# QEC-project-2020/MCMC-QEC-toric-RL

Measured on AMD Instinct MI355X. Metric: MCMC sweeps/sec (whole node), L=9 toric p=0.15; eq-class histogram match, higher is better.
Workload: dtype u8

## Files before the change

mcmc-qec-toric-rl_amd/csrc/ladder_wu.hpp:

```cpp
#pragma once
#include "ladder_kernel.hpp"
#include "shortest_book.hpp"
#include "wu_frames.hpp"

namespace qecmc {

constexpr uint32_t kWuPickStream = 0x800u;
constexpr uint32_t kSubWuPick = 9u, kSubWuAcc = 10u, kSubWuRefine = 11u;

#ifndef QECMC_WU_PRIO_SHIFT
#define QECMC_WU_PRIO_SHIFT 4
#endif
constexpr int kWuPrioShift = QECMC_WU_PRIO_SHIFT;
constexpr bool wu_prio_family(int WV, bool ALPHA) { return kWuPrioShift >= 0 && !ALPHA && WV <= 16; }
__device__ __forceinline__ void wu_step_priority(uint32_t t)
{
    constexpr uint32_t SH = kWuPrioShift < 0 ? 0u : (uint32_t)kWuPrioShift;
    uint32_t k;
    asm volatile("s_and_b32 %0, %1, %2\n\t"
                 "s_cmp_lg_u32 %0, 0\n\t"
                 "s_cbranch_scc1 4f\n\t"
                 "s_bfe_u32 %0, %1, %3\n\t"
                 "s_cmp_lg_u32 %0, 0\n\t"
                 "s_cbranch_scc1 1f\n\t"
                 "s_setprio 3\n\t"
                 "s_branch 4f\n"
                 "1:\n\t"
                 "s_cmp_lg_u32 %0, 1\n\t"
                 "s_cbranch_scc1 2f\n\t"
                 "s_setprio 2\n\t"
                 "s_branch 4f\n"
                 "2:\n\t"
                 "s_cmp_lg_u32 %0, 2\n\t"
                 "s_cbranch_scc1 3f\n\t"
                 "s_setprio 1\n\t"
                 "s_branch 4f\n"
                 "3:\n\t"
                 "s_setprio 0\n"
                 "4:"
                 : "=&s"(k) : "s"(t), "n"((1u << SH) - 1u), "n"(SH | (2u << 16)) : "scc");
}

template <int WV> struct WuVec;
template <> struct WuVec<4> { typedef uint32_t type __attribute__((ext_vector_type(4))); };
template <> struct WuVec<8> { typedef uint32_t type __attribute__((ext_vector_type(8))); };
template <> struct WuVec<12> { typedef uint32_t type __attribute__((ext_vector_type(12))); };
template <> struct WuVec<16> { typedef uint32_t type __attribute__((ext_vector_type(16))); };
template <> struct WuVec<32> { typedef uint32_t type __attribute__((ext_vector_type(32))); };

template <int WV> constexpr int wu_base() { return WV == 32 ? 48 : 64 - WV; }
#define WU_BY_WV(M)                                                                                                            \
    if constexpr (WV == 4) { M("{v[60:63]}") } else if constexpr (WV == 8) { M("{v[56:63]}") }                                 \
    else if constexpr (WV == 12) { M("{v[52:63]}") } else if constexpr (WV == 16) { M("{v[48:63]}") }                          \
    else { static_assert(WV == 32, "state widths: 4, 8, 12, 16, 32 words"); M("{v[48:79]}") }
#define WU_EACH(M) M(0) M(1) M(2) M(3) M(4) M(5) M(6) M(7) M(8) M(9) M(10) M(11) M(12) M(13) M(14) M(15) \
                   M(16) M(17) M(18) M(19) M(20) M(21) M(22) M(23) M(24) M(25) M(26) M(27) M(28) M(29) M(30) M(31)

template <int WV> __device__ __forceinline__ void wu_def(typename WuVec<WV>::type &st)
{
#define M(PIN) asm volatile("" : "=" PIN(st));
    WU_BY_WV(M)
#undef M
}
template <int WV> __device__ __forceinline__ void wu_pin(typename WuVec<WV>::type &st)
{
#define M(PIN) asm volatile("" : "+" PIN(st));
    WU_BY_WV(M)
#undef M
}
template <int WV, int w> __device__ __forceinline__ void wu_set(typename WuVec<WV>::type &st, uint32_t v)
{
#define M(PIN) asm volatile("v_mov_b32 v[%c[r]], %[v]" : "+" PIN(st) : [r] "i"(wu_base<WV>() + w), [v] "v"(v));
    WU_BY_WV(M)
#undef M
}
template <int WV, int w> __device__ __forceinline__ uint32_t wu_get(typename WuVec<WV>::type &st)
{
    uint32_t v;
#define M(PIN) asm volatile("v_mov_b32 %[v], v[%c[r]]" : [v] "=v"(v), "+" PIN(st) : [r] "i"(wu_base<WV>() + w));
    WU_BY_WV(M)
#undef M
    return v;
}
template <int WV, int w> __device__ __forceinline__ void wu_xor_s(typename WuVec<WV>::type &st, uint32_t m)
{
// ... 241 lines not shown
    if (xf < ef - band) return true;
    if (xf > ef + band) return false;
    return (double)x * (1.0 / 4294967296.0) < det_exp(y);
}

struct WuAl { uint32_t Dh, any, Nb; };

template <int CODE, int WV>
__device__ __forceinline__ void wu_propose_alpha(const LadderArgs &a, typename WuVec<WV>::type &st, WuAl &al, uint32_t a12, uint32_t cht_addr,
                                                 float lxy, float lz, uint32_t d0, uint32_t d1, uint32_t d2, uint32_t d3,
                                                 uint32_t x0, uint32_t x1, uint32_t x2, uint32_t x3, uint32_t tlo, uint32_t thi, uint32_t omask, uint32_t amask,
                                                 uint64_t refine_k, uint32_t refine_w, uint32_t syn, uint32_t slot, uint32_t m55)
{
    const uint32_t F = wu_read<WV>(st, d0, d1, d2, d3);
    const uint32_t pv = __builtin_amdgcn_perm(thi, tlo, (F & amask) | omask);
    const uint32_t addr = __builtin_amdgcn_sad_u8(pv, 0u, cht_addr);
    const uint32_t dch = *(wu_lds_ptr)(uintptr_t)addr;
    const wu_half2 pD = __builtin_bit_cast(wu_half2, al.Dh) + __builtin_bit_cast(wu_half2, dch);
    const float e = __builtin_amdgcn_exp2f(__builtin_fmaf((float)pD.x, lxy, __builtin_fmaf((float)pD.y, lz, 12.0f)));
    const float dm = e - (float)a12;
    bool acc = dm >= 2.0f;
    if (!acc && dm >= -1.0f) {
        const int nq = a.nq, T1 = nq + 1;
        const double *bt = a.bias_tbl + (size_t)slot * 4 * T1;
        uint32_t nxc = 0;
#define QECMC_WU_CX(w) if constexpr (w < WV) wu_count_x<WV, w>(st, nxc, m55);
        WU_EACH(QECMC_WU_CX)
#undef QECMC_WU_CX
        int dx = 0;
        {
            const uint32_t P0 = x0 >> ((d0 >> 8) & 31u), P1 = x1 >> ((d1 >> 8) & 31u), P2 = x2 >> ((d2 >> 8) & 31u), P3 = x3 >> ((d3 >> 8) & 31u);
            const uint32_t f0 = F & 3u, f1 = (F >> 8) & 3u, f2 = (F >> 16) & 3u, f3 = (F >> 24) & 3u;
            dx += (int)((f0 ^ P0) == 1u) - (int)(f0 == 1u);
            dx += (int)((f1 ^ P1) == 1u) - (int)(f1 == 1u);
            dx += (int)((f2 ^ P2) == 1u) - (int)(f2 == 1u);
            dx += (int)((f3 ^ P3) == 1u) - (int)(f3 == 1u);
        }
        const int bx = (int)(al.Nb & 1023u), bz = (int)((al.Nb >> 10) & 1023u), bxy = (int)(al.Nb >> 20);
        const int cx = (int)nxc + dx, cz = bz + (int)(float)pD.y, cxy = bxy + (int)(float)pD.x;
        const double pn = bt[cx] * bt[T1 + (cxy - cx)] * bt[2 * T1 + cz] * bt[3 * T1 + (nq - cxy - cz)];
        const double pb = bt[bx] * bt[T1 + (bxy - bx)] * bt[2 * T1 + bz] * bt[3 * T1 + (nq - bxy - bz)];
        const double ratio = pn / pb;
        const double ulo = (double)a12 * (1.0 / 4096.0);
        acc = ulo + (1.0 / 4096.0) <= ratio;
        if (!acc && ulo < ratio) {
            const u32x4 rb = wu_philox(refine_k, kSubWuRefine, syn, slot, a.seed_lo, a.seed_hi);
            const uint64_t v44 = ((uint64_t)a12 << 32) | sel4(rb, (int)refine_w);
            acc = (double)v44 * (1.0 / 17592186044416.0) < ratio;
        }
    }
    if (acc) {
        wu_xor<WV>(st, d0, d1, d2, d3, x0, x1, x2, x3);
        al.Dh = __builtin_bit_cast(uint32_t, pD);
        al.any = 1u;
    }
}

template <int CODE>
__device__ __forceinline__ void wu_stage_lds(const LadderArgs &a, uint64_t lad, uint32_t slot, wu_lds_rw xrow, uint32_t &n4, uint32_t &cls, int w0 = 0, int w1 = -1, int rows = 0)
{
    const int NC = a.Nc, W = a.W, L = a.L, nq = a.nq;
    const uint8_t *src = a.resume ? a.states + (lad * NC + slot) * (uint64_t)nq : a.init + (lad / a.replicas) * (uint64_t)nq;
    uint32_t cnt = 0;
    if (w1 < 0) w1 = W;
#pragma unroll 1
    for (int w = w0; w < w1; ++w) {
        uint32_t word = 0;
#pragma unroll 4
        for (int b = 0; b < 16; ++b) {
            const int cell = w * 8 + (b >> 1), q = CODE == kCodeToric ? (cell < L * L ? (b & 1) * L * L + cell : nq) : w * 16 + b;
            if (q < nq) word |= (uint32_t)(src[q] & 3u) << (2 * b);
        }
        xrow[(w - w0) * 64] = word;
        cnt += nnz2(word);
    }
#pragma unroll 1
    for (int r = w1 - w0; r < rows; ++r) xrow[r * 64] = 0u;
    if (w0 != 0) { n4 += 4u * cnt; return; }
    n4 = 4u * cnt;
    cls = (uint32_t)(CODE == kCodeToric ? toric_eq_class_b(L, src) : surf_eq_class_b(CODE, L, src));
    if (CODE == kCodeXzzx) cls = cls == 0 ? 0u : cls == 1 ? 1u : cls == 2 ? 3u : 2u;
}

__device__ __forceinline__ bool wu_pair_flips(const LadderArgs &a, uint32_t car, uint32_t lo, uint32_t x, uint32_t trow, int i)
{
    const int d = (int)(car & 0xFFFFu) - (int)(lo & 0xFFFFu);
    const int dt = d < 0 ? 0 : d > kSwapFast - 1 ? kSwapFast - 1 : d;
    uint32_t thr = *(wu_lds_ptr)(uintptr_t)(trow + 4u * (uint32_t)dt);
    if (__builtin_amdgcn_sicmp(d, kSwapFast - 1, 38) != 0) {
        int il = i, nql = a.nq;
        asm volatile("" : "+s"(il), "+s"(nql));
        const int dg = d < 0 ? 0 : d > nql ? nql : d;
        const uint32_t far = (uint32_t)a.swap_thr[(size_t)il * (size_t)(nql + 1) + (size_t)dg];
        thr = d >= kSwapFast ? far : thr;
    }
    return d <= 0 || x < thr;
}

template <int CODE, int WV, bool CONV, bool QUEUE, bool TOP, int IT, bool ALPHA, bool STATS = false, bool SHORT = false, bool LONG = true>
__device__ __forceinline__ void wu_run(const LadderArgs &a, typename WuVec<WV>::type &st, WuCtx &cx, const WuEnv &ev)
{
    static_assert(!QUEUE || CONV, "the work queue serves the runs that stop by the criterion");
    static_assert(!ALPHA || CODE != kCodeToric, "the alpha rule: xzzx / rotated codes");
    static_assert(!STATS || (!CONV && WV <= 16), "the statistics kernels: fixed-length runs of up to 16 state words");
    static_assert(!SHORT || (CONV && QUEUE && ALPHA && !STATS), "the shortest-chain kernels: the alpha rule's queue kernels");
    [[maybe_unused]] uint32_t swapc = 0, nsum = 0;
    const int L = a.L;
    wu_lds_ptr const lml = (wu_lds_ptr)(uintptr_t)(ev.lds0 + ev.lml_off);
    const uint32_t lds0 = ev.lds0, slot = ev.slot, grp = ev.grp;
    const int lane = ev.lane;
    constexpr bool top = TOP;
    constexpr bool LEAN = !CONV && !ALPHA && WV <= 16;
    constexpr bool FRAME = TOP && wu_frame_steps(WV, CONV, ALPHA, IT) != 0;
    constexpr uint32_t FW = (uint32_t)WV + 1u;
    const uint32_t G = a.n_gen;
    const uint32_t m55 = 0x55555555u;
    uint32_t n4 = cx.n4, cls = cx.cls, flag = cx.flag;
    [[maybe_unused]] uint32_t nef = cx.nef;
    [[maybe_unused]] float lxyf = 0.0f, lzf = 0.0f;
    if constexpr (ALPHA) { lxyf = a.bias_l2f[ev.slot][0]; lzf = a.bias_l2f[ev.slot][1]; }
    [[maybe_unused]] const uint32_t cht_base = ev.lds0 + ev.cht_off;
    uint32_t syn = a.first_syndrome + ev.lad;
    [[maybe_unused]] uint32_t t0 = 0;
    [[maybe_unused]] uint32_t tops0 = cx.tops0, samples = 0;
    const wu_const_ptr desc = (wu_const_ptr)a.wu_desc;
    const uint32_t iters = IT ? (uint32_t)IT : a.iters;
    const uint32_t nch = (iters + 9u) / 10u, nc4 = (iters + 3u) / 4u;
    const uint32_t S = 128u / iters;
    const uint32_t thr16 = (uint32_t)((a.thr_logical + 65535u) >> 16);
    const uint32_t thr_base = lds0 + ev.thr_off;
    uint32_t nbias = 0u - (thr_base + 16u);
    asm volatile("" : "+s"(nbias));
    uint32_t pk = 0;
    [[maybe_unused]] uint32_t pa0 = 0, pa1 = 0, pb0 = 0, pb1 = 0;
    [[maybe_unused]] uint32_t pf_a = 0, pf_b = 0, pf_c = 0, pf_l = 0;
    uint32_t ws = (uint32_t)(a.step0 % S);
    uint64_t wi = a.step0 / S;
    auto refresh = [&]() {
        const u32x4 b = wu_philox(wi * 64u + (uint64_t)lane, kSubWuPick, grp, kWuPickStream + slot, a.seed_lo, a.seed_hi);
        if constexpr (FRAME) {
            constexpr uint32_t FS = (uint32_t)wu_frame_steps(WV, CONV, ALPHA, IT);
            wu_lds_rw const frm = (wu_lds_rw)(uintptr_t)(lds0 + ev.frm_off);
#pragma unroll
            for (uint32_t i = 0; i < (FS * FW + 63u) / 64u; ++i) {
                const uint32_t at = i * 64u + (uint32_t)lane;
                if (at < FS * FW) frm[at] = 0u;
            }
            __builtin_amdgcn_fence(__ATOMIC_ACQ_REL, "wavefront");
            if ((uint32_t)lane < FS * (uint32_t)IT / 2u) {
                wu_lds_rw const row = frm + ((uint32_t)lane / ((uint32_t)IT / 2u)) * FW;
                auto desc_word = [&](uint32_t g, int i) { return a.wu_desc[(size_t)g * (CODE == kCodeToric ? 8u : 16u) + (uint32_t)i]; };
                auto lml_word = [&](uint32_t kind, uint32_t pos, int w) { return lml[(kind * (uint32_t)(L + 1) + pos) * (uint32_t)WV + (uint32_t)w]; };
                auto xor_word = [&](uint32_t w, uint32_t v) { __hip_atomic_fetch_xor(row + w, v, __ATOMIC_RELAXED, __HIP_MEMORY_SCOPE_WORKGROUP); };
                wu_frame_add<CODE, WV>(b.x, b.y, thr16, G, L, desc_word, lml_word, xor_word);
                wu_frame_add<CODE, WV>(b.z, b.w, thr16, G, L, desc_word, lml_word, xor_word);
            }
            __builtin_amdgcn_fence(__ATOMIC_ACQ_REL, "wavefront");
        } else {
        const uint32_t g0 = scale_u32(b.y, G), g1 = scale_u32(b.w, G);
        pk = CODE == kCodeToric ? (g0 << 5) | (g1 << 21) : (g0 << 6) | (g1 << 22);
        if (top) { pa0 = b.x; pb0 = b.y; pa1 = b.z; pb1 = b.w; }
        }
    };
    refresh();
    constexpr bool AHEAD = LEAN && !TOP && IT == 10;
    [[maybe_unused]] u32x4 abn{0, 0, 0, 0};
    if constexpr (AHEAD) abn = wu_philox(a.step0, kSubWuAcc, syn, slot, a.seed_lo, a.seed_hi);

    for (uint64_t t = 0; QUEUE || t < a.nsteps + (CONV ? 1u : 0u); ++t) {
        if constexpr (wu_prio_family(WV, ALPHA)) wu_step_priority((uint32_t)t);
        const uint64_t T = QUEUE ? (uint64_t)((uint32_t)t - t0) : a.step0 + t;
        [[maybe_unused]] uint32_t maskv = 0, cdelta = 0;
        const uint32_t pbase = ws * iters;
        [[maybe_unused]] WuAl al{0u, 0u, 0u};
        if constexpr (ALPHA && !top) al.Nb = wu_counts_packed<WV>(st, m55, a.W);
        if constexpr (FRAME) {
            const uint32_t fv = ((wu_lds_ptr)(uintptr_t)(lds0 + ev.frm_off))[ws * FW + (uint32_t)(lane < WV ? lane : WV)];
            maskv = fv;
            cdelta = (uint32_t)__builtin_amdgcn_readlane((int)fv, WV);
// ... 44 lines not shown
#undef QECMC_WU_LOGICAL
                } else {
                    const uint32_t j = c * 10u + (uint32_t)f;
                    if constexpr (IT == 10) {
                        if constexpr (ALPHA) {
                          if ((f & 1) == 0) {
                            const wu_const_ptr eb = (wu_const_ptr)((wu_const_bytes)desc + (r >> 16));
                            const uint32_t d0 = e[0], d1 = e[1], d2 = e[2], d3 = e[3], x0 = e[4], x1 = e[5], x2 = e[6], x3 = e[7];
                            const uint32_t am = e[11], tlo = e[12], thi = e[13], om = e[14], coff = e[15];
                            const uint32_t b0 = eb[0], b1 = eb[1], b2 = eb[2], b3 = eb[3], y0 = eb[4], y1 = eb[5], y2 = eb[6], y3 = eb[7];
                            const uint32_t an = eb[11], ulo = eb[12], uhi = eb[13], on = eb[14], cofn = eb[15];
                            __builtin_amdgcn_sched_barrier(0);
                            wu_propose_alpha<CODE, WV>(a, st, al, wu_field(ab, f), cht_base + coff, lxyf, lzf, d0, d1, d2, d3, x0, x1, x2, x3, tlo, thi, om, am,
                                                       T * nc4 + (j >> 2), j & 3u, syn, slot, m55);
                            wu_propose_alpha<CODE, WV>(a, st, al, wu_field(ab, f + 1), cht_base + cofn, lxyf, lzf, b0, b1, b2, b3, y0, y1, y2, y3, ulo, uhi, on, an,
                                                       T * nc4 + ((j + 1u) >> 2), (j + 1u) & 3u, syn, slot, m55);
                          }
                        } else if constexpr (CODE == kCodeToric) {
                          if ((f & 1) == 0) {
                            const wu_desc8 da = *(wu_const_desc8)e, db = *(wu_const_desc8)((wu_const_bytes)desc + (r >> 16));
                            __builtin_amdgcn_sched_barrier(0);
                            wu_propose<CODE, WV>(st, n4, wu_field(ab, f), thr_base, nbias, da[0], 0u, da[1], da[2], da[3], 0u, da[4], da[5], da[6], 0u, 0u, 0u,
                                                 T * nc4 + (j >> 2), j & 3u, syn, slot, a.seed_lo, a.seed_hi);
                            wu_propose<CODE, WV>(st, n4, wu_field(ab, f + 1), thr_base, nbias, db[0], 0u, db[1], db[2], db[3], 0u, db[4], db[5], db[6], 0u, 0u, 0u,
                                                 T * nc4 + ((j + 1u) >> 2), (j + 1u) & 3u, syn, slot, a.seed_lo, a.seed_hi);
                          }
                        } else
                        if ((f & 1) == 0) {
                            const wu_const_ptr eb = (wu_const_ptr)((wu_const_bytes)desc + (r >> 16));
                            const uint32_t d0 = e[0], d1 = e[1], d2 = e[2], d3 = e[3], x0 = e[4], x1 = e[5], x2 = e[6], x3 = e[7], tlo = e[8];
                            const uint32_t thi = e[9], om = e[10], am = e[11];
                            const uint32_t b0 = eb[0], b1 = eb[1], b2 = eb[2], b3 = eb[3], y0 = eb[4], y1 = eb[5], y2 = eb[6], y3 = eb[7], ulo = eb[8];
                            const uint32_t uhi = eb[9], on = eb[10], an = eb[11];
                            __builtin_amdgcn_sched_barrier(0);
                            wu_propose<CODE, WV>(st, n4, wu_field(ab, f), thr_base, nbias, d0, d1, d2, d3, x0, x1, x2, x3, tlo, thi, om, am,
                                                 T * nc4 + (j >> 2), j & 3u, syn, slot, a.seed_lo, a.seed_hi);
                            wu_propose<CODE, WV>(st, n4, wu_field(ab, f + 1), thr_base, nbias, b0, b1, b2, b3, y0, y1, y2, y3, ulo, uhi, on, an,
                                                 T * nc4 + ((j + 1u) >> 2), (j + 1u) & 3u, syn, slot, a.seed_lo, a.seed_hi);
                        }
                    } else if constexpr (ALPHA) {
                        const uint32_t d0 = e[0], d1 = e[1], d2 = e[2], d3 = e[3], x0 = e[4], x1 = e[5], x2 = e[6], x3 = e[7];
                        const uint32_t am = e[11], tlo = e[12], thi = e[13], om = e[14], coff = e[15];
                        wu_propose_alpha<CODE, WV>(a, st, al, wu_field(ab, f), cht_base + coff, lxyf, lzf, d0, d1, d2, d3, x0, x1, x2, x3, tlo, thi, om, am,
                                                   T * nc4 + (j >> 2), j & 3u, syn, slot, m55);
                    } else if constexpr (CODE == kCodeToric) {
                        const wu_desc8 d = *(wu_const_desc8)e;
                        wu_propose<CODE, WV>(st, n4, wu_field(ab, f), thr_base, nbias, d[0], 0u, d[1], d[2], d[3], 0u, d[4], d[5], d[6], 0u, 0u, 0u,
                                             T * nc4 + (j >> 2), j & 3u, syn, slot, a.seed_lo, a.seed_hi);
                    } else {
                        const uint32_t d0 = e[0], d1 = e[1], d2 = e[2], d3 = e[3], x0 = e[4], x1 = e[5], x2 = e[6], x3 = e[7], tlo = e[8];
                        const uint32_t thi = e[9], om = e[10], am = e[11];
                        wu_propose<CODE, WV>(st, n4, wu_field(ab, f), thr_base, nbias, d0, d1, d2, d3, x0, x1, x2, x3, tlo, thi, om, am,
                                             T * nc4 + (j >> 2), j & 3u, syn, slot, a.seed_lo, a.seed_hi);
                    }
                }
            }
        }
        if (top) {
            cls ^= cdelta;
            n4 = 0;
            [[maybe_unused]] uint32_t tx = 0, tz = 0, txy = 0;
#define QECMC_WU_FLUSH(w)                                                                                    \
            if constexpr (w < WV) {                                                                          \
                wu_xor_s<WV, w>(st, (uint32_t)__builtin_amdgcn_readlane((int)maskv, w));                     \
                if constexpr (ALPHA) wu_count3<WV, w>(st, tx, tz, txy, m55);                                 \
                else wu_count<WV, w>(st, n4, m55);                                                           \
            }
            WU_EACH(QECMC_WU_FLUSH)
#undef QECMC_WU_FLUSH
            if constexpr (ALPHA) { n4 = tz + txy; nef = tz | (txy << 16); }
            n4 <<= 2;
        } else if constexpr (ALPHA) {
            const wu_half2 D = __builtin_bit_cast(wu_half2, al.Dh);
            const uint32_t ez = (uint32_t)((int)((al.Nb >> 10) & 1023u) + (int)(float)D.y), exy = (uint32_t)((int)(al.Nb >> 20) + (int)(float)D.x);
            n4 = (ez + exy) << 2;
            if (al.any) nef = ez | (exy << 16);
        }
        if (++ws == S) { ws = 0; ++wi; refresh(); }

        if constexpr (LEAN) {
        int NCl = a.Nc, ncl = a.ncls;
        uint32_t slotl = ev.slot, lds0l = ev.lds0, once = a.wu_once;
        asm volatile("" : "+s"(NCl), "+s"(ncl), "+s"(slotl), "+s"(lds0l), "+s"(once));
        if constexpr (STATS) once = 0;
        const int NC = NCl;
        const uint32_t slot = slotl;
        const WuLds ol = wu_lds(NC, WV, ncl, 0, false, false);
        constexpr uint32_t xstride = (uint32_t)WV * 256u;
        const uint32_t xaddr = lds0l + (uint32_t)lane * 4u;
        wu_lds_rw const recl = (wu_lds_rw)(uintptr_t)(xaddr + (uint32_t)ol.rec * 4u), swdl = recl + NC * 64;
        const uint32_t tb0 = lds0l + (uint32_t)ol.swapT * 4u;
        const int swb = NC - 1 - (int)slot;
        constexpr bool TOPDRAWS = !LONG && wu_frame_steps(WV, CONV, ALPHA, IT) != 0;
        u32x4 sb{0, 0, 0, 0};
        [[maybe_unused]] u32x4 sb1{0, 0, 0, 0};
        [[maybe_unused]] bool duty = false;
        if constexpr (TOPDRAWS && TOP) {
            sb = wu_philox(T, 0u, syn, kSwapStream, a.seed_lo, a.seed_hi);
            if (NC > 5) sb1 = wu_philox(T, 1u, syn, kSwapStream, a.seed_lo, a.seed_hi);
        } else if constexpr (!TOPDRAWS) {
            duty = swb >= 0 && swb < 4 && swb * 4 < NC - 1;
            if (duty) sb = wu_philox(T, (uint32_t)swb, syn, kSwapStream, a.seed_lo, a.seed_hi);
        }
        auto put_block = [&](int blk, const u32x4 &v) {
            wu_lds_rw p = swdl + (uint32_t)(blk * 4) * 64u;
            const int left = NC - 1 - blk * 4;
            p[0] = v.x;
            if (left > 1) p[64] = v.y;
            if (left > 2) p[128] = v.z;
            if (left > 3) p[192] = v.w;
        };
        __syncthreads();
        wu_put_all<WV>(st, xaddr + slot * xstride);
        recl[slot * 64u] = pack_info(n4 >> 2, slot, cls, flag);
        if constexpr (TOPDRAWS && TOP) {
            put_block(0, sb);
            if (NC > 5) put_block(1, sb1);
        } else if constexpr (!TOPDRAWS) {
            if (duty) put_block(swb, sb);
        }
        wu_ds_wait<WV>(st);
        __syncthreads();
        if constexpr (AHEAD) {
            abn = wu_philox(T + 1u, kSubWuAcc, syn, slot, a.seed_lo, a.seed_hi);
            asm volatile("" : "+v"(abn.x), "+v"(abn.y), "+v"(abn.z), "+v"(abn.w));
        }
        uint32_t mine;
        if (once) {
            if constexpr (TOP) {
                wu_lds_rw pr = recl + (NC - 2) * 64, px = swdl + (NC - 2) * 64;
                uint32_t trow = tb0 + (uint32_t)(NC - 2) * (uint32_t)(kSwapFast * 4);
                uint32_t car = pr[64], lo = pr[0], x = px[0];
                for (int i = NC - 2; i >= 0; --i) {
                    const uint32_t lo_n = pr[-64], x_n = px[-64];
                    const bool flip = wu_pair_flips(a, car, lo, x, trow, i);
                    pr[64] = flip ? lo : car;
                    car = flip ? car : lo;
                    lo = lo_n; x = x_n; pr -= 64; px -= 64; trow -= (uint32_t)(kSwapFast * 4);
                }
                pr[64] = car;
            }
            __syncthreads();
            mine = recl[slot * 64u];
        } else {
            wu_lds_ptr pr = recl + (NC - 2) * 64, px = swdl + (NC - 2) * 64;
            uint32_t trow = tb0 + (uint32_t)(NC - 2) * (uint32_t)(kSwapFast * 4);
            uint32_t car = pr[64];
            for (int i = NC - 2; i >= (int)slot; --i) {
                const uint32_t lo = pr[0];
                car = wu_pair_flips(a, car, lo, px[0], trow, i) ? car : lo;
                pr -= 64; px -= 64; trow -= (uint32_t)(kSwapFast * 4);
            }
            mine = car;
            if (slot != 0) {
                const uint32_t lo = pr[0];
                if (wu_pair_flips(a, car, lo, px[0], trow, (int)slot - 1)) {
                    mine = lo;
                    if constexpr (STATS) swapc += 1u;
                }
            }
        }
        wu_take_all<WV>(st, xaddr + ((mine >> 16) & 0xFFu) * xstride);
        n4 = (mine & 0xFFFFu) << 2; cls = (mine >> 24) & 0x3Fu; flag = mine >> 31;
        if constexpr (STATS) nsum += mine & 0xFFFFu;
        if (top) flag = 1;
        if (slot == 0) {
            tops0 += (NC == 1) | flag;
            if (a.counts != nullptr && tops0 >= a.tops_burn) {
                wu_lds_rw const hist = (wu_lds_rw)(uintptr_t)(xaddr + (uint32_t)ol.hist * 4u);
                hist[(CODE == kCodeXzzx ? (cls ^ (cls >> 1)) : cls) * 64] += 1;
                samples++;
            }
            flag = 0;
        }
        } else {
        int NCl = a.Nc, nql = a.nq, ncl = a.ncls, Ll = a.L, Wl = a.W;
        uint32_t slotl = ev.slot, lds0l = ev.lds0;
        asm volatile("" : "+s"(NCl), "+s"(nql), "+s"(ncl), "+s"(Ll), "+s"(slotl), "+s"(lds0l), "+s"(Wl));
        const int NC = NCl, nq = nql, ncls = ncl;
        const uint32_t slot = slotl;
        const WuLds ol = wu_lds(NC, Wl, ncls, Ll, CONV, ALPHA, SHORT);
        wu_lds_rw const ldsl = (wu_lds_rw)(uintptr_t)lds0l;
        wu_lds_rw const rec = ldsl + ol.rec, swd = ldsl + ol.swd, hist = ldsl + ol.hist, swapT = ldsl + ol.swapT;
        volatile __attribute__((address_space(3))) uint32_t *const stopf = ldsl + ol.stop;
        [[maybe_unused]] wu_lds_rw const bk = ldsl + ol.bk + (uint32_t)lane, mail = ldsl + ol.mail, bot = ldsl + ol.bot, bot2 = ldsl + ol.bot2;
        [[maybe_unused]] wu_lds_drw const nefd = (wu_lds_drw)(ldsl + ol.nef) + (uint32_t)lane;
        [[maybe_unused]] wu_lds_dptr const lnbd = (wu_lds_dptr)(ldsl + ol.lnb);
        [[maybe_unused]] wu_lds_rw const skey = ldsl + ol.skey + (uint32_t)lane, sst = ldsl + ol.sst + (uint32_t)lane;
        const uint32_t xaddr = lds0l + (uint32_t)lane * 4u;
        constexpr bool PAD = WV == 32 || !CONV;
        const uint32_t xstride = (uint32_t)(WV == 32 ? kWuHalf : PAD ? WV : Wl) * 256u;
        const int swb = NC - 1 - (int)slot;
        u32x4 sb{0, 0, 0, 0};
        const bool duty = swb >= 0 && swb < 4 && swb * 4 < NC - 1;
        if (duty) sb = wu_philox(T, (uint32_t)swb, syn, kSwapStream, a.seed_lo, a.seed_hi);
        __syncthreads();
        {
            const uint32_t xo = xaddr + slot * xstride;
#define QECMC_WU_PUT(w) if constexpr (w < WV && w < kWuHalf) { if (WV == 32 || !CONV || w < wu_words_min(WV) || w < Wl) wu_ds_write<WV, w>(st, xo); }
#define QECMC_WU_PUT_HI(w) if constexpr (w < WV && w >= kWuHalf) wu_ds_write<WV, w, w - kWuHalf>(st, xo);
            WU_EACH(QECMC_WU_PUT)
            rec[slot * 64u + (uint32_t)lane] = pack_info(n4 >> 2, slot, cls, flag);
            if constexpr (ALPHA) nefd[slot * 64u] = alpha_neff(nef, a.alpha);
            if (duty) {
                wu_lds_rw p = swd + (uint32_t)(swb * 4) * 64u + (uint32_t)lane;
                const int left = NC - 1 - swb * 4;
                p[0] = sb.x;
                if (left > 1) p[64] = sb.y;
                if (left > 2) p[128] = sb.z;
                if (left > 3) p[192] = sb.w;
            }
        }
        wu_ds_wait<WV>(st);
        __syncthreads();
        if constexpr (CONV) { if (stopf[t & 1]) break; }
        {
            wu_lds_ptr cur = rec + (uint32_t)lane, sx = swd + (uint32_t)lane;
            uint32_t car = cur[(NC - 1) * 64], mine = car;
            const int i_stop = slot == 0 ? 0 : (int)slot - 1;
            for (int i = NC - 2; i >= i_stop; --i) {
                const uint32_t lo = cur[i * 64], x = sx[i * 64];
                bool flip;
                if constexpr (ALPHA) {
                    flip = wu_alpha_flip(x, nefd[(i + 1) * 64], nefd[i * 64], lnbd[i]);
                } else {
                const int d = (int)(car & 0xFFFFu) - (int)(lo & 0xFFFFu);
                const int dd = d < 1 ? 1 : d;
                bool lt = x < swapT[i * kSwapFast + (dd < kSwapFast ? dd : 0)];
                if (dd >= kSwapFast) lt = (uint64_t)x < a.swap_thr[(size_t)i * (nq + 1) + dd];
                flip = d <= 0 || lt;
                }
                const uint32_t into = flip ? lo : car;
                car = flip ? car : lo;
                if ((int)slot == i + 1) {
                    mine = into;
                    if constexpr (STATS) swapc += flip ? 1u : 0u;
                }
            }
            if (slot == 0) mine = car;
// ... 230 lines not shown
```

mcmc-qec-toric-rl_amd/csrc/tables_test_api.cpp:

```cpp
#include "class_sweep.hpp"
#include "class_sweep_cut.hpp"
#include "class_sweep_tiled.hpp"
#include "class_sweep_site.hpp"
#include "class_minplus.hpp"
#include "class_minplus_trace.hpp"
#include "class_minplus_site.hpp"
#include "class_minplus_tiled.hpp"
#include "corrections.hpp"
#include "enumerate.hpp"
#include "kernel_choice.hpp"
#include "plan_host.hpp"
#include "syndrome_lift.hpp"
#include "tables.hpp"
#include "wu_frames.hpp"

#include <cstdio>
#include <cstring>

using namespace qecmc;
using namespace qecmc::tables;

namespace {
template <class T> int put(const std::vector<T> &v, T *out, int cap)
{
    if ((int)v.size() > cap) return -(int)v.size();
    std::memcpy(out, v.data(), v.size() * sizeof(T));
    return (int)v.size();
}
int answer(const Refusal &r, const KernelShape &s, int32_t *shape_ints, char *msg, int msg_cap)
{
    if (msg && msg_cap > 0) std::snprintf(msg, (size_t)msg_cap, "%s", r.msg.c_str());
    if (!r.code && shape_ints) std::memcpy(shape_ints, &s, sizeof s);
    return r.code;
}
std::vector<uint32_t> gen_table(int code, int L) { return code == QECMC_TORIC ? toric_generator_table(L) : surf_generator_table(code, L); }
}

extern "C" {
int qt_generator_table(int code, int L, uint32_t *out, int cap) { return put(gen_table(code, L), out, cap); }
int qt_logical_masks(int code, int L, int W, uint32_t *out, int cap)
{
    return put(code == QECMC_TORIC ? toric_logical_masks(L, W) : surf_logical_masks(code, L, W), out, cap);
}
int qt_wave_descriptors(int code, int L, uint32_t *out, int cap) { return put(wave_descriptors(gen_table(code, L)), out, cap); }
uint32_t qt_wave_position(int code, int L, uint32_t q) { return wave_position(code, L, q); }
int qt_toric_wave_descriptors(int L, uint32_t *out, int cap) { return put(toric_wave_descriptors(toric_generator_table(L)), out, cap); }
int qt_wave_logical_masks(int code, int L, int W, uint32_t *out, int cap)
{
    const std::vector<uint32_t> flat = code == QECMC_TORIC ? toric_logical_masks(L, W) : surf_logical_masks(code, L, W);
    return put(wave_layout_rows(code, L, (int)code_nq(code, L), W, flat), out, cap);
}
int qt_plan_wave_tables(const qecmc_params *p, uint32_t *desc, int desc_cap, int *n_desc, uint32_t *lmask, int lmask_cap, int *n_lmask)
{
    HostPlan hp;
    if (validate_params(p).code || plan_host(*p, hp).code) return -1;
    *n_desc = put(hp.wu_desc, desc, desc_cap);
    *n_lmask = put(hp.lmask, lmask, lmask_cap);
    return *n_desc < 0 || *n_lmask < 0 ? -1 : 0;
}
uint64_t qt_thr64(double v) { return thr64(v); }
uint64_t qt_thr44(double v) { return thr44(v); }
uint32_t qt_thr32(double v) { return thr32(v); }
double qt_chain_factor(double p) { return chain_factor(p); }
int qt_ladder(double p_bottom, double p_top, int Nc, double *pl, double *pd)
{
    std::vector<double> a, b;
    ladder_probabilities(p_bottom, p_top, Nc, a, b);
    std::memcpy(pl, a.data(), a.size() * sizeof(double));
    if (!b.empty()) std::memcpy(pd, b.data(), b.size() * sizeof(double));
    return (int)b.size();
}
int qt_bias_tables(int alpha_model, double p, double eta_or_alpha, int nq, double *out, int cap)
{
    return put(alpha_model ? alpha_tables(p, eta_or_alpha, (size_t)nq) : bias_tables(p, eta_or_alpha, (size_t)nq), out, cap);
}
int qt_patterns(int code, int L, uint8_t *gen_type, int cap_types, uint32_t *patterns, int cap_patterns)
{
    std::vector<uint8_t> gt;
    std::vector<uint32_t> pat;
    generator_patterns(gen_table(code, L), gt, pat);
    if (put(gt, gen_type, cap_types) < 0) return -1;
    return put(pat, patterns, cap_patterns);
}
int qt_count_change(const uint32_t *patterns, int n, uint32_t *out, int cap)
{
    return put(count_change_table(std::vector<uint32_t>(patterns, patterns + n)), out, cap);
}
int qt_swap_thresholds(const double *pdiff, int n, int nq, uint64_t *out, int cap)
{
    return put(swap_thresholds(std::vector<double>(pdiff, pdiff + n), nq), out, cap);
}
int qt_colour_phases(int code, int L, uint16_t *out, int cap)
{
    int n_phases = 0;
    const std::vector<uint16_t> ph = colour_phases(gen_table(code, L), n_phases);
    return put(ph, out, cap) < 0 ? -1 : n_phases;
// ... 323 lines not shown
}
int qt_class_minplus_trace_plan(int code, int L, int lds_width, int32_t *forget_gen, uint32_t *forget_words, int cap_words, int32_t *out4)
{
    const minplus::TracePlan tp = minplus::build_trace_plan(code, L, lds_width);
    if (tp.cut.plan.refusal.code || (int)tp.forget_words.size() > cap_words) return -1;
    for (int i = 0; i < tp.n_forget; ++i) forget_gen[i] = tp.forget_gen[(size_t)i];
    if (!tp.forget_words.empty()) std::memcpy(forget_words, tp.forget_words.data(), tp.forget_words.size() * sizeof(uint32_t));
    if (out4) { out4[0] = tp.n_forget; out4[1] = tp.words_per_forget; out4[2] = tp.cut.plan.W; out4[3] = (int32_t)minplus::trace_bytes_per_pair(tp); }
    return tp.n_forget;
}
uint32_t qt_class_minplus_trace_group(uint64_t N, int ncls, int n_held, uint64_t bytes_per_pair, uint64_t *workspace)
{
    if (workspace) *workspace = minplus::kTraceWorkspaceBytes;
    return minplus::trace_launch_group(N, ncls, n_held, bytes_per_pair);
}
int qt_class_minplus_site(int code, int L, uint64_t N, const uint8_t *chains, const uint8_t *cq, uint64_t cq_rows, int lds_width, uint32_t *cost_out, uint64_t *count_out,
                          int32_t *cls, char *msg, int msg_cap)
{
    if (!chains || !cq || !cost_out || !count_out) return site_answer(refuse_params(QECMC_ERR_INVALID, "qecmc_class_minplus_site: NULL buffer"), msg, msg_cap);
    if (N > 0xFFFFFFFFull) return site_answer(refuse_params(QECMC_ERR_INVALID, "qecmc_class_minplus_site: N=%llu syndromes exceed 32 bits", (unsigned long long)N), msg, msg_cap);
    const sweep::CutPlan cp = minplus::build_minplus_site_plan(code, L, lds_width);
    if (cp.plan.refusal.code) return site_answer(cp.plan.refusal, msg, msg_cap);
    if (const Refusal r = minplus::check_cost_rows("qecmc_class_minplus_site", N, cq_rows); r.code) return site_answer(r, msg, msg_cap);
    minplus::minplus_cut_site_host(cp, N, chains, cq, cq_rows, cost_out, count_out, cls);
    return site_answer({}, msg, msg_cap);
}
int qt_class_minplus_chains_site(int code, int L, uint64_t N, const uint8_t *chains, const uint8_t *cq, uint64_t cq_rows, int lds_width, uint8_t *chain_out, uint32_t *cost_out,
                                 uint64_t *count_out, int32_t *cls, char *msg, int msg_cap)
{
    if (!chains || !cq || !chain_out) return site_answer(refuse_params(QECMC_ERR_INVALID, "qecmc_class_minplus_chains_site: NULL buffer"), msg, msg_cap);
    if (N > 0xFFFFFFFFull)
        return site_answer(refuse_params(QECMC_ERR_INVALID, "qecmc_class_minplus_chains_site: N=%llu syndromes exceed 32 bits", (unsigned long long)N), msg, msg_cap);
    const minplus::TracePlan tp = minplus::build_trace_site_plan(code, L, lds_width);
    if (tp.cut.plan.refusal.code) return site_answer(tp.cut.plan.refusal, msg, msg_cap);
    if (const Refusal r = minplus::check_cost_rows("qecmc_class_minplus_chains_site", N, cq_rows); r.code) return site_answer(r, msg, msg_cap);
    minplus::minplus_trace_site_host(tp, N, chains, cq, cq_rows, chain_out, cost_out, count_out, cls);
    return site_answer({}, msg, msg_cap);
}
void qt_site_cost_words(const uint8_t *cq, uint64_t rows, int nq, uint32_t *out) { minplus::site_cost_words(cq, rows, nq, out); }
int qt_class_minplus_tiled(int code, int L, uint64_t N, const uint8_t *chains, const uint32_t *cost, int hbm_width, int tile_width, uint32_t *cost_out, uint64_t *count_out,
                           int32_t *cls, char *msg, int msg_cap)
{
    if (!chains || !cost || !cost_out || !count_out) return site_answer(refuse_params(QECMC_ERR_INVALID, "qecmc_class_minplus_tiled: NULL buffer"), msg, msg_cap);
    if (N > 0xFFFFFFFFull) return site_answer(refuse_params(QECMC_ERR_INVALID, "qecmc_class_minplus_tiled: N=%llu syndromes exceed 32 bits", (unsigned long long)N), msg, msg_cap);
    if (const Refusal r = minplus::check_tiled_costs(cost); r.code) return site_answer(r, msg, msg_cap);
    const sweep::TiledPlan tp = minplus::build_minplus_tiled_plan(code, L, hbm_width, tile_width, "qecmc_class_minplus_tiled");
    if (tp.plan.refusal.code) return site_answer(tp.plan.refusal, msg, msg_cap);
    if (const Refusal r = minplus::check_tiled_cost_range(tp.plan, cost); r.code) return site_answer(r, msg, msg_cap);
    minplus::minplus_tiled_host(tp, N, chains, cost, cost_out, count_out, cls);
    return site_answer({}, msg, msg_cap);
}
int qt_class_minplus_tiled_site(int code, int L, uint64_t N, const uint8_t *chains, const uint8_t *cq, uint64_t cq_rows, int hbm_width, int tile_width, uint32_t *cost_out,
                                uint64_t *count_out, int32_t *cls, char *msg, int msg_cap)
{
    if (!chains || !cq || !cost_out || !count_out) return site_answer(refuse_params(QECMC_ERR_INVALID, "qecmc_class_minplus_tiled_site: NULL buffer"), msg, msg_cap);
    if (N > 0xFFFFFFFFull)
        return site_answer(refuse_params(QECMC_ERR_INVALID, "qecmc_class_minplus_tiled_site: N=%llu syndromes exceed 32 bits", (unsigned long long)N), msg, msg_cap);
    const sweep::TiledPlan tp = minplus::build_minplus_tiled_plan(code, L, hbm_width, tile_width, "qecmc_class_minplus_tiled_site");
    if (tp.plan.refusal.code) return site_answer(tp.plan.refusal, msg, msg_cap);
    if (const Refusal r = minplus::check_cost_rows("qecmc_class_minplus_tiled_site", N, cq_rows); r.code) return site_answer(r, msg, msg_cap);
    if (N > 0)
        if (const Refusal r = minplus::check_tiled_cost_rows_range(cq, cq_rows, tp.plan.nq, sweep::closed_qubits(tp.ops, tp.plan.nq)); r.code) return site_answer(r, msg, msg_cap);
    minplus::minplus_tiled_site_host(tp, N, chains, cq, cq_rows, cost_out, count_out, cls);
    return site_answer({}, msg, msg_cap);
}
int qt_wave_frames(const qecmc_params *p, const uint32_t *picks, uint32_t *frames, int cap)
{
    HostPlan hp;
    if (validate_params(p).code || plan_host(*p, hp).code || p->scan != QECMC_SCAN_WAVE) return -1;
    const LadderArgs &a = hp.args;
    const int L = a.L, W = a.W, WV = wu_words(W);
    const uint32_t steps = 128u / a.iters, thr16 = (uint32_t)((a.thr_logical + 65535u) >> 16);
    if (WV > 16 || (int)(steps * (uint32_t)(WV + 1)) > cap) return -1;
    std::vector<uint32_t> lml((size_t)4 * (L + 1) * WV, 0u);
    for (int row = 0; row < 4 * (L + 1); ++row)
        for (int w = 0; w < W; ++w) lml[(size_t)row * WV + w] = hp.lmask[(size_t)row * W + w];
#define QT_FRAMES(CODE, WVC) if (a.code == CODE && WV == WVC) wu_build_frames<CODE, WVC>(picks, a.iters, thr16, a.n_gen, L, hp.wu_desc.data(), lml.data(), frames);
#define QT_FRAMES_W(CODE) QT_FRAMES(CODE, 4) QT_FRAMES(CODE, 8) QT_FRAMES(CODE, 12) QT_FRAMES(CODE, 16)
    QT_FRAMES_W(kCodeToric) QT_FRAMES_W(kCodeXzzx) QT_FRAMES_W(kCodeRotated) QT_FRAMES_W(kCodePlanar)
#undef QT_FRAMES_W
#undef QT_FRAMES
    return WV;
}
}
```

Before: 8.014 billion.

## Precompute per-pair swap bounds from uniforms before the replica-exchange scan

Each replica-exchange uniform is turned once into an integer bound on the weight difference, before the draws are written to LDS. A log2-based first guess is checked against the near threshold row, with a fallback walk over the global table. The serial swap scan then only does integer compares of weight differences against that bound, with no per-pair threshold loads. The TOP path gains an unrolled 8-replica register version, and LONG kernels are forced off the one-pass path. This adds transcendental and LDS work per draw and assumes the bound exactly matches the old threshold comparison.

```diff
diff --git a/mcmc-qec-toric-rl_amd/csrc/ladder_wu.hpp b/mcmc-qec-toric-rl_amd/csrc/ladder_wu.hpp
--- a/mcmc-qec-toric-rl_amd/csrc/ladder_wu.hpp
+++ b/mcmc-qec-toric-rl_amd/csrc/ladder_wu.hpp
@@ -1,6 +1,7 @@
 #pragma once
 #include "ladder_kernel.hpp"
 #include "shortest_book.hpp"
+#include "wu_bounds.hpp"
 #include "wu_frames.hpp"
 
 namespace qecmc {
@@ -408,19 +409,36 @@
     if (CODE == kCodeXzzx) cls = cls == 0 ? 0u : cls == 1 ? 1u : cls == 2 ? 3u : 2u;
 }
 
-__device__ __forceinline__ bool wu_pair_flips(const LadderArgs &a, uint32_t car, uint32_t lo, uint32_t x, uint32_t trow, int i)
-{
-    const int d = (int)(car & 0xFFFFu) - (int)(lo & 0xFFFFu);
-    const int dt = d < 0 ? 0 : d > kSwapFast - 1 ? kSwapFast - 1 : d;
-    uint32_t thr = *(wu_lds_ptr)(uintptr_t)(trow + 4u * (uint32_t)dt);
-    if (__builtin_amdgcn_sicmp(d, kSwapFast - 1, 38) != 0) {
-        int il = i, nql = a.nq;
-        asm volatile("" : "+s"(il), "+s"(nql));
-        const int dg = d < 0 ? 0 : d > nql ? nql : d;
-        const uint32_t far = (uint32_t)a.swap_thr[(size_t)il * (size_t)(nql + 1) + (size_t)dg];
-        thr = d >= kSwapFast ? far : thr;
-    }
-    return d <= 0 || x < thr;
+__device__ __forceinline__ void wu_bound_block(const LadderArgs &a, u32x4 &v, uint32_t trow, int i0, int left)
+{
+    int nql = a.nq;
+    asm volatile("" : "+s"(nql));
+    constexpr uint32_t RB = (uint32_t)(kSwapFast * 4);
+    auto near = [&](uint32_t row) { return [row](int d) { return *(wu_lds_ptr)(uintptr_t)(row + 4u * (uint32_t)d); }; };
+    uint32_t g0 = 0, g1 = 0, g2 = 0, g3 = 0;
+    bool ok = true, ok1 = true, ok2 = true, ok3 = true;
+    if (left > 2) {
+        g0 = wu_swap_first(v.x, a.swap_inv_log2[i0], nql); g1 = wu_swap_first(v.y, a.swap_inv_log2[i0 + 1], nql);
+        g2 = wu_swap_first(v.z, a.swap_inv_log2[i0 + 2], nql); g3 = wu_swap_first(v.w, a.swap_inv_log2[i0 + 3], nql);
+        uint32_t a0 = near(trow)((int)g0), b0 = near(trow)((int)g0 + 1), a1 = near(trow + RB)((int)g1), b1 = near(trow + RB)((int)g1 + 1);
+        uint32_t a2 = near(trow + 2u * RB)((int)g2), b2 = near(trow + 2u * RB)((int)g2 + 1), a3 = near(trow + 3u * RB)((int)g3), b3 = near(trow + 3u * RB)((int)g3 + 1);
+        asm volatile("" : "+v"(a0), "+v"(b0), "+v"(a1), "+v"(b1), "+v"(a2), "+v"(b2), "+v"(a3), "+v"(b3));
+        ok = wu_swap_holds(v.x, a0, b0); ok1 = wu_swap_holds(v.y, a1, b1); ok2 = wu_swap_holds(v.z, a2, b2);
+        ok3 = left == 3 || wu_swap_holds(v.w, a3, b3);
+    } else {
+        ok = wu_swap_guess(v.x, a.swap_inv_log2[i0], nql, near(trow), g0);
+        if (left > 1) ok1 = wu_swap_guess(v.y, a.swap_inv_log2[i0 + 1], nql, near(trow + RB), g1);
+    }
+    if (__builtin_amdgcn_ballot_w64(!(ok && ok1 && ok2 && ok3)) != 0) {
+        int il = i0;
+        asm volatile("" : "+s"(il));
+        auto far = [&](int k) { return [&a, il, nql, k](int d) { return (uint32_t)a.swap_thr[(size_t)(il + k) * (size_t)(nql + 1) + (size_t)d]; }; };
+        if (!ok) g0 = wu_swap_walk(v.x, g0, nql, near(trow), far(0));
+        if (!ok1) g1 = wu_swap_walk(v.y, g1, nql, near(trow + RB), far(1));
+        if (!ok2) g2 = wu_swap_walk(v.z, g2, nql, near(trow + 2u * RB), far(2));
+        if (!ok3) g3 = wu_swap_walk(v.w, g3, nql, near(trow + 3u * RB), far(3));
+    }
+    v.x = g0; v.y = g1; v.z = g2; v.w = g3;
 }
 
 template <int CODE, int WV, bool CONV, bool QUEUE, bool TOP, int IT, bool ALPHA, bool STATS = false, bool SHORT = false, bool LONG = true>
@@ -631,7 +649,7 @@
         int NCl = a.Nc, ncl = a.ncls;
         uint32_t slotl = ev.slot, lds0l = ev.lds0, once = a.wu_once;
         asm volatile("" : "+s"(NCl), "+s"(ncl), "+s"(slotl), "+s"(lds0l), "+s"(once));
-        if constexpr (STATS) once = 0;
+        if constexpr (STATS || LONG) once = 0;
         const int NC = NCl;
         const uint32_t slot = slotl;
         const WuLds ol = wu_lds(NC, WV, ncl, 0, false, false);
@@ -644,12 +662,18 @@
         u32x4 sb{0, 0, 0, 0};
         [[maybe_unused]] u32x4 sb1{0, 0, 0, 0};
         [[maybe_unused]] bool duty = false;
+        auto bound_block = [&](int blk, u32x4 &v) { wu_bound_block(a, v, tb0 + (uint32_t)(blk * 4) * (uint32_t)(kSwapFast * 4), blk * 4, NC - 1 - blk * 4); };
         if constexpr (TOPDRAWS && TOP) {
             sb = wu_philox(T, 0u, syn, kSwapStream, a.seed_lo, a.seed_hi);
             if (NC > 5) sb1 = wu_philox(T, 1u, syn, kSwapStream, a.seed_lo, a.seed_hi);
+            bound_block(0, sb);
+            if (NC > 5) bound_block(1, sb1);
         } else if constexpr (!TOPDRAWS) {
             duty = swb >= 0 && swb < 4 && swb * 4 < NC - 1;
-            if (duty) sb = wu_philox(T, (uint32_t)swb, syn, kSwapStream, a.seed_lo, a.seed_hi);
+            if (duty) {
+                sb = wu_philox(T, (uint32_t)swb, syn, kSwapStream, a.seed_lo, a.seed_hi);
+                bound_block(swb, sb);
+            }
         }
         auto put_block = [&](int blk, const u32x4 &v) {
             wu_lds_rw p = swdl + (uint32_t)(blk * 4) * 64u;
@@ -676,34 +700,45 @@
         }
         uint32_t mine;
         if (once) {
-            if constexpr (TOP) {
-                wu_lds_rw pr = recl + (NC - 2) * 64, px = swdl + (NC - 2) * 64;
-                uint32_t trow = tb0 + (uint32_t)(NC - 2) * (uint32_t)(kSwapFast * 4);
-                uint32_t car = pr[64], lo = pr[0], x = px[0];
-                for (int i = NC - 2; i >= 0; --i) {
-                    const uint32_t lo_n = pr[-64], x_n = px[-64];
-                    const bool flip = wu_pair_flips(a, car, lo, x, trow, i);
-                    pr[64] = flip ? lo : car;
-                    car = flip ? car : lo;
-                    lo = lo_n; x = x_n; pr -= 64; px -= 64; trow -= (uint32_t)(kSwapFast * 4);
+            if constexpr (TOP && !LONG) {
+                wu_lds_rw const pr = recl + (NC - 8) * 64;
+                wu_lds_ptr const px = swdl + (NC - 8) * 64;
+                uint32_t r[8], s[7];
+#pragma unroll
+                for (int j = 0; j < 8; ++j) r[j] = pr[64 * (7 - j)];
+#pragma unroll
+                for (int j = 0; j < 7; ++j) s[j] = px[64 * (6 - j)];
+                asm volatile("" : "+v"(r[0]), "+v"(r[1]), "+v"(r[2]), "+v"(r[3]), "+v"(r[4]), "+v"(r[5]), "+v"(r[6]), "+v"(r[7]),
+                                  "+v"(s[0]), "+v"(s[1]), "+v"(s[2]), "+v"(s[3]), "+v"(s[4]), "+v"(s[5]), "+v"(s[6]));
+#pragma unroll
+                for (int j = 0; j < 7; ++j) s[j] += r[j + 1] & 0xFFFFu;
+                uint32_t car = r[0], nc = car & 0xFFFFu;
+#pragma unroll
+                for (int j = 0; j < 7; ++j) {
+                    if (j < NC - 1) {
+                        const uint32_t lo = r[j + 1];
+                        const bool flip = nc <= s[j];
+                        pr[64 * (7 - j)] = flip ? lo : car;
+                        car = flip ? car : lo;
+                        nc = flip ? nc : lo & 0xFFFFu;
+                    }
                 }
-                pr[64] = car;
+                recl[0] = car;
             }
             __syncthreads();
             mine = recl[slot * 64u];
         } else {
             wu_lds_ptr pr = recl + (NC - 2) * 64, px = swdl + (NC - 2) * 64;
-            uint32_t trow = tb0 + (uint32_t)(NC - 2) * (uint32_t)(kSwapFast * 4);
             uint32_t car = pr[64];
             for (int i = NC - 2; i >= (int)slot; --i) {
                 const uint32_t lo = pr[0];
-                car = wu_pair_flips(a, car, lo, px[0], trow, i) ? car : lo;
-                pr -= 64; px -= 64; trow -= (uint32_t)(kSwapFast * 4);
+                car = wu_bound_flips(car, lo, px[0]) ? car : lo;
+                pr -= 64; px -= 64;
             }
             mine = car;
             if (slot != 0) {
                 const uint32_t lo = pr[0];
-                if (wu_pair_flips(a, car, lo, px[0], trow, (int)slot - 1)) {
+                if (wu_bound_flips(car, lo, px[0])) {
                     mine = lo;
                     if constexpr (STATS) swapc += 1u;
                 }
diff --git a/mcmc-qec-toric-rl_amd/csrc/tables_test_api.cpp b/mcmc-qec-toric-rl_amd/csrc/tables_test_api.cpp
--- a/mcmc-qec-toric-rl_amd/csrc/tables_test_api.cpp
+++ b/mcmc-qec-toric-rl_amd/csrc/tables_test_api.cpp
@@ -12,6 +12,7 @@
 #include "plan_host.hpp"
 #include "syndrome_lift.hpp"
 #include "tables.hpp"
+#include "wu_bounds.hpp"
 #include "wu_frames.hpp"
 
 #include <cstdio>
@@ -501,4 +502,27 @@
 #undef QT_FRAMES
     return WV;
 }
-}
+int qt_wave_swap_bound(const qecmc_params *p, int pair, const uint32_t *xs, uint64_t n, uint32_t *out)
+{
+    HostPlan hp;
+    if (validate_params(p).code || plan_host(*p, hp).code || p->scan != QECMC_SCAN_WAVE || p->noise != QECMC_NOISE_DEPOLARIZING) return -1;
+    const LadderArgs &a = hp.args;
+    if (pair < 0 || pair + 1 >= a.Nc || !a.swap_fast_ok) return -1;
+    const int nq = a.nq;
+    const uint64_t *thr = hp.swap_thr.data() + (size_t)pair * (nq + 1);
+    uint32_t row[kSwapFast];
+    for (int d = 0; d < kSwapFast; ++d) row[d] = (d >= 1 && d <= nq) ? (uint32_t)thr[d] : 0u;
+    for (uint64_t k = 0; k < n; ++k)
+        out[k] = wu_swap_bound(xs[k], a.swap_inv_log2[pair], nq, [&](int d) { return row[d]; }, [&](int d) { return (uint32_t)thr[d]; });
+    return nq;
+}
+int qt_wave_swap_row(const qecmc_params *p, int pair, uint64_t *out, int cap)
+{
+    HostPlan hp;
+    if (validate_params(p).code || plan_host(*p, hp).code || p->scan != QECMC_SCAN_WAVE) return -1;
+    const LadderArgs &a = hp.args;
+    if (pair < 0 || pair + 1 >= a.Nc || cap < a.nq + 1) return -1;
+    for (int d = 0; d <= a.nq; ++d) out[d] = hp.swap_thr[(size_t)pair * (a.nq + 1) + d];
+    return a.nq + 1;
+}
+}
diff --git a/mcmc-qec-toric-rl_amd/csrc/wu_bounds.hpp b/mcmc-qec-toric-rl_amd/csrc/wu_bounds.hpp
--- /dev/null
+++ b/mcmc-qec-toric-rl_amd/csrc/wu_bounds.hpp
@@ -0,0 +1,51 @@
+#pragma once
+#include <math.h>
+#include <stdint.h>
+
+#include "kernel_choice.hpp"
+
+namespace qecmc {
+
+__host__ __device__ __forceinline__ uint32_t wu_swap_first(uint32_t x, float inv, int nq)
+{
+#if defined(__HIP_DEVICE_COMPILE__)
+    const float l2 = __log2f((float)x + 0.5f);
+#else
+    const float l2 = log2f((float)x + 0.5f);
+#endif
+    const int hi = nq < kSwapFast - 2 ? nq : kSwapFast - 2;
+    const float r = (l2 - 32.0f) * inv;
+    return (uint32_t)(int)fminf(fmaxf(r, 0.0f), (float)hi);
+}
+__host__ __device__ __forceinline__ bool wu_swap_holds(uint32_t x, uint32_t t0, uint32_t t1) { return x - t1 < t0 - t1; }
+template <class Near>
+__host__ __device__ __forceinline__ bool wu_swap_guess(uint32_t x, float inv, int nq, Near &&near, uint32_t &g)
+{
+    g = wu_swap_first(x, inv, nq);
+    return wu_swap_holds(x, near((int)g), near((int)g + 1));
+}
+
+template <class Near, class Far>
+__host__ __device__ __forceinline__ uint32_t wu_swap_walk(uint32_t x, uint32_t start, int nq, Near &&near, Far &&far)
+{
+    auto below = [&](int dd) -> bool { return dd < kSwapFast ? x < near(dd) : x < far(dd); };
+    int d = (int)start;
+    while (d < nq && below(d + 1)) ++d;
+    while (d > 0 && !below(d)) --d;
+    return (uint32_t)d;
+}
+
+template <class Near, class Far>
+__host__ __device__ __forceinline__ uint32_t wu_swap_bound(uint32_t x, float inv, int nq, Near &&near, Far &&far)
+{
+    uint32_t g;
+    if (wu_swap_guess(x, inv, nq, near, g)) return g;
+    return wu_swap_walk(x, g, nq, near, far);
+}
+
+__host__ __device__ __forceinline__ bool wu_bound_flips(uint32_t car, uint32_t lo, uint32_t bound)
+{
+    return (int)(car & 0xFFFFu) - (int)(lo & 0xFFFFu) <= (int)bound;
+}
+
+}
```

Result: faster. 8.126 billion, median of 6 (+1.4%).
